# FofanovLab/mtsv_tools

Measured on AMD Instinct MI355X. Metric: reads/sec (whole node), 150bp reads vs MG-index, higher is better.
Workload: dtype u32/i16

## Files before the change

mtsv_tools_amd/csrc/dev_index.hip:

```cpp
#include <algorithm>
#include <chrono>
#include <cstdio>
#include <cstdlib>
#include <cstring>
#include <stdexcept>
#include <thread>
#include <vector>

#include "dev_index.hpp"
#include "kernels.hpp"

namespace mtsv {

void throw_hip(hipError_t e, const char* what, const char* file, int line) {
    throw std::runtime_error(std::string("device: ") + hipGetErrorString(e) + " at " + what + " (" + file + ":" +
                             std::to_string(line) + ")");
}

DeviceIndex::~DeviceIndex() {
    if (device < 0) return;
    (void)hipSetDevice(device);
    (void)hipFree(d_blocks);
    (void)hipFree(d_sa_sample);
    (void)hipFree(d_sa_full);
    (void)hipFree(d_text);
    (void)hipFree(d_bin_end);
    (void)hipFree(d_bins);
    (void)hipFree(d_bin_lut);
    (void)hipFree(d_kmer);
    (void)hipFree(d_kmer_levels);
}

namespace {

inline uint32_t sym_code(uint8_t c) {
    switch (c) {
    case 'A': return kCodeA;
    case 'C': return kCodeC;
    case 'G': return kCodeG;
    case 'T': return kCodeT;
    case 'N': return kCodeN;
    case '$': return kCodeSentinel;
    default: return 7;
    }
}


__global__ void k_expand_sa(DevIndexView ix, uint32_t n_samples, uint32_t* __restrict__ sa_full) {
    uint32_t j = blockIdx.x * blockDim.x + threadIdx.x;
    if (j >= n_samples) return;
    uint32_t row = j * ix.sa_s;
    uint32_t v = ix.sa_sample[j];
    sa_full[row] = v;
    for (uint32_t guard = 0; guard <= ix.n; guard++) {
        uint32_t blk = row >> kBlockShift, off = row & (kBlockRows - 1);
        LoadedBlock b = load_block(ix.blocks, blk);
        uint32_t c = block_code(b, off);
        if (c == kCodeSentinel) break;
        row = less_of(ix, c) + block_rank(b, c, blk, off, ix.sentinel_row);
        v -= 1;
        if (row % ix.sa_s == 0) break;
        sa_full[row] = v;
    }
}

__global__ void k_kmer_level1(DevIndexView ix, uint2* __restrict__ tab) {
    uint32_t a = threadIdx.x;
    if (a >= 4) return;
    uint32_t lo = less_of(ix, a) + dev_rank(ix, a, 0);
    uint32_t hi = less_of(ix, a) + dev_rank(ix, a, ix.n);
    tab[a] = make_uint2(lo, hi);
}

__global__ void k_kmer_level(DevIndexView ix, const uint2* __restrict__ prev, uint2* __restrict__ cur,
                             uint32_t prev_shift) {
    const uint64_t total = 4ull << prev_shift, stride = (uint64_t)gridDim.x * blockDim.x;
    for (uint64_t t = (uint64_t)blockIdx.x * blockDim.x + threadIdx.x; t < total; t += stride) {
        uint32_t a = (uint32_t)(t >> prev_shift);
        uint64_t p = t & ((1ull << prev_shift) - 1);
        uint2 iv = prev[p];
        uint32_t lo = 0, hi = 0;
        if (iv.x < iv.y) {
            uint32_t b0 = iv.x >> kBlockShift, b1 = iv.y >> kBlockShift;
            LoadedBlock B0 = load_block(ix.blocks, b0);
            lo = less_of(ix, a) + block_rank(B0, a, b0, iv.x & (kBlockRows - 1), ix.sentinel_row);
            if (b1 == b0) {
                hi = less_of(ix, a) + block_rank(B0, a, b1, iv.y & (kBlockRows - 1), ix.sentinel_row);
            } else {
                LoadedBlock B1 = load_block(ix.blocks, b1);
                hi = less_of(ix, a) + block_rank(B1, a, b1, iv.y & (kBlockRows - 1), ix.sentinel_row);
            }
        }
        cur[t] = make_uint2(lo, hi);
    }
}

__global__ void k_kmer_tag(DevIndexView ix, uint2* __restrict__ tab, uint64_t total, unsigned long long* __restrict__ n_tagged) {
    const uint64_t stride = (uint64_t)gridDim.x * blockDim.x;
    uint32_t mine = 0;
    for (uint64_t t = (uint64_t)blockIdx.x * blockDim.x + threadIdx.x; t < total; t += stride) {
        const uint2 iv = tab[t];
        if (iv.y != iv.x + 1) continue;
        const uint32_t lo = iv.x;
        const uint32_t p = ix.sa_full[lo];
        const LoadedBlock b = load_block(ix.blocks, lo >> kBlockShift);
        const uint32_t c1 = block_code(b, lo & (kBlockRows - 1));
        const uint32_t c2 = p >= 2 ? ix.text[p - 2] : 7u;
        tab[t] = kmer_tag_entry(p, c1, c2);
        mine++;
    }
    for (int d = 32; d > 0; d >>= 1) mine += __shfl_down(mine, d);
    if ((threadIdx.x & 63) == 0 && mine) atomicAdd(n_tagged, (unsigned long long)mine);
}

template <class F>
void parallel_ranges(uint64_t n, int threads, F fn) {
    std::vector<std::thread> pool;
    uint64_t chunk = (n + threads - 1) / threads;
    for (int t = 0; t < threads; t++) {
        uint64_t lo = std::min(n, (uint64_t)t * chunk), hi = std::min(n, lo + chunk);
        pool.emplace_back(fn, lo, hi, t);
    }
    for (auto& th : pool) th.join();
}

}

static void pack_on_host(const HostIndex& hx, const uint32_t n, const uint32_t n_blocks, std::vector<RankBlock>& blocks, uint64_t& sentinel_row,
                         std::vector<uint8_t>& codes) {
    int threads = (int)std::max(1u, std::min(32u, std::thread::hardware_concurrency()));
    if (n_blocks < 4096) threads = 1;

    blocks.resize(n_blocks);
    std::vector<std::array<uint64_t, 6>> range_cnt(threads);
    uint64_t blocks_per = ((uint64_t)n_blocks + threads - 1) / threads;
    parallel_ranges(n_blocks, threads, [&](uint64_t, uint64_t, int t) {
        uint64_t b0 = std::min<uint64_t>(n_blocks, (uint64_t)t * blocks_per), b1 = std::min<uint64_t>(n_blocks, b0 + blocks_per);
        std::array<uint64_t, 6> c{};
        uint64_t lo = b0 << kBlockShift, hi = std::min<uint64_t>(n, b1 << kBlockShift);
        for (uint64_t i = lo; i < hi; i++) {
            uint32_t code = sym_code(hx.bwt[i]);
            if (code < 6) c[code]++;
        }
        range_cnt[t] = c;
    });
    std::vector<std::array<uint64_t, 6>> range_base(threads);
    {
        std::array<uint64_t, 6> acc{};
        for (int t = 0; t < threads; t++) {
            range_base[t] = acc;
            for (int a = 0; a < 6; a++) acc[a] += range_cnt[t][a];
        }
    }
    std::vector<std::string> errs(threads);
    std::vector<uint64_t> sentinel_rows(threads, UINT64_MAX);
    static const uint8_t syms[6] = {'A', 'C', 'G', 'T', 'N', '$'};
    parallel_ranges(n_blocks, threads, [&](uint64_t, uint64_t, int t) {
        uint64_t b0 = std::min<uint64_t>(n_blocks, (uint64_t)t * blocks_per), b1 = std::min<uint64_t>(n_blocks, b0 + blocks_per);
        std::array<uint64_t, 6> c = range_base[t];
        for (uint64_t b = b0; b < b1; b++) {
            RankBlock rb;
            for (int a = 0; a < 4; a++) rb.cnt[a] = (uint32_t)c[a];
            uint64_t p0[2] = {0, 0}, p1[2] = {0, 0}, p2[2] = {0, 0};
            for (uint32_t o = 0; o < kBlockRows; o++) {
                uint64_t i = (b << kBlockShift) + o;
                uint32_t code = 7;
                if (i < n) {
                    code = sym_code(hx.bwt[i]);
                    if (code >= 6) {
                        errs[t] = "format: bwt holds a symbol outside ACGTN$";
                        return;
                    }
                    c[code]++;
                    if (code == kCodeSentinel) sentinel_rows[t] = i;
                    if (i % hx.k == 0) {
                        uint64_t j = i / hx.k;
                        for (int a = 0; a < 6; a++)
                            if (hx.occ[syms[a]][j] != c[a]) {
                                errs[t] = "format: Occ checkpoint " + std::to_string(j) + " disagrees with the bwt";
                                return;
                            }
                    }
                }
                p0[o >> 6] |= (uint64_t)(code & 1) << (o & 63);
                p1[o >> 6] |= (uint64_t)((code >> 1) & 1) << (o & 63);
                p2[o >> 6] |= (uint64_t)((code >> 2) & 1) << (o & 63);
            }
            rb.p0[0] = p0[0]; rb.p0[1] = p0[1];
            rb.p1[0] = p1[0]; rb.p1[1] = p1[1];
            rb.p2[0] = p2[0]; rb.p2[1] = p2[1];
            blocks[b] = rb;
        }
    });
    for (auto& e : errs)
        if (!e.empty()) throw std::runtime_error(e);
    sentinel_row = UINT64_MAX;
    for (uint64_t s : sentinel_rows)
        if (s != UINT64_MAX) sentinel_row = s;
    if (sentinel_row == UINT64_MAX) throw std::runtime_error("format: bwt holds no sentinel");

    codes.assign(((uint64_t)n + 15) / 16 * 16 + 32, (uint8_t)7);
    parallel_ranges(n, threads, [&](uint64_t lo, uint64_t hi, int) {
        for (uint64_t i = lo; i < hi; i++) codes[i] = (uint8_t)sym_code(hx.text[i]);
    });
}

namespace {
struct DevTemp {
    void* p = nullptr;
    ~DevTemp() { (void)hipFree(p); }
    void alloc(uint64_t bytes) { HIP_CHECK(hipMalloc(&p, bytes ? bytes : 16)); }
    void release() {
        HIP_CHECK(hipFree(p));
        p = nullptr;
    }
};
struct DevEvents {
    hipEvent_t e[7] = {nullptr, nullptr, nullptr, nullptr, nullptr, nullptr, nullptr};
    DevEvents() {
        for (auto& x : e) HIP_CHECK(hipEventCreate(&x));
    }
    ~DevEvents() {
        for (auto& x : e)
            if (x) (void)hipEventDestroy(x);
    }
};
}

static uint64_t pack_on_device(const HostIndex& hx, const uint32_t n, const uint32_t n_blocks, DeviceIndex& di, double& copy_ms) {
    auto now_ms = [] { return std::chrono::duration<double, std::milli>(std::chrono::steady_clock::now().time_since_epoch()).count(); };
    uint32_t tile = kPackTile;
    if (const char* e = getenv("MTSV_PACK_TILE")) {
        const int t = atoi(e);
        if (t >= 1 && t <= (int)kPackTileMax && !(t & (t - 1))) tile = (uint32_t)t;
    }
    static const uint8_t syms[6] = {'A', 'C', 'G', 'T', 'N', '$'};
    const uint64_t n_chk = ((uint64_t)n - 1) / hx.k + 1;
    for (uint8_t a : syms)
        if (hx.occ[a].size() < n_chk) throw std::runtime_error("format: occ checkpoint count != floor((n-1)/k)+1");
    const uint32_t tiles = pack_tiles(n_blocks, tile);
    const uint64_t raw_bytes = ((uint64_t)n + 15) / 16 * 16;
    DevEvents ev;
    DevTemp d_bwt, d_occ, d_tiles, d_ctr, d_raw_text;

    HIP_CHECK(hipMalloc((void**)&di.d_blocks, (uint64_t)n_blocks * sizeof(RankBlock)));
    di.bytes += (uint64_t)n_blocks * sizeof(RankBlock);
    d_bwt.alloc(raw_bytes);
    d_occ.alloc(6 * n_chk * 8);
    d_tiles.alloc((uint64_t)tiles * sizeof(uint4));
    d_ctr.alloc(kPackCounters * 4);
    uint32_t ctr[kPackCounters] = {0};
    ctr[kPackCtrForeignRow] = ctr[kPackCtrOccBadFirst] = 0xffffffffu;
    double t0 = now_ms();
    HIP_CHECK(hipMemcpy(d_bwt.p, hx.bwt.data(), n, hipMemcpyHostToDevice));
    for (int a = 0; a < 6; a++)
        HIP_CHECK(hipMemcpy((uint64_t*)d_occ.p + a * n_chk, hx.occ[syms[a]].data(), n_chk * 8, hipMemcpyHostToDevice));
    HIP_CHECK(hipMemcpy(d_ctr.p, ctr, sizeof ctr, hipMemcpyHostToDevice));
    copy_ms += now_ms() - t0;

    HIP_CHECK(hipEventRecord(ev.e[0], 0));
    launch_pack_count(0, (const uint8_t*)d_bwt.p, n, n_blocks, tile, (uint4*)d_tiles.p, (uint32_t*)d_ctr.p);
    HIP_CHECK(hipEventRecord(ev.e[1], 0));
    launch_pack_scan(0, (uint4*)d_tiles.p, tiles);
    HIP_CHECK(hipEventRecord(ev.e[2], 0));
    launch_pack_blocks(0, (const uint8_t*)d_bwt.p, n, n_blocks, tile, (const uint4*)d_tiles.p, di.d_blocks);
    HIP_CHECK(hipEventRecord(ev.e[3], 0));
    launch_pack_check_occ(0, di.d_blocks, n, hx.k, (uint32_t)n_chk, (const uint64_t*)d_occ.p, (uint32_t*)d_ctr.p);
    HIP_CHECK(hipGetLastError());
    HIP_CHECK(hipEventRecord(ev.e[4], 0));
    HIP_CHECK(hipMemcpy(ctr, d_ctr.p, sizeof ctr, hipMemcpyDeviceToHost));
    d_bwt.release();
    d_occ.release();
    d_tiles.release();
    d_ctr.release();
    const uint64_t occ_row = ctr[kPackCtrOccBad] ? (uint64_t)ctr[kPackCtrOccBadFirst] * hx.k : UINT64_MAX;
    if (ctr[kPackCtrForeign] && ctr[kPackCtrForeignRow] <= occ_row) throw std::runtime_error("format: bwt holds a symbol outside ACGTN$");
    if (ctr[kPackCtrOccBad])
        throw std::runtime_error("format: Occ checkpoint " + std::to_string(ctr[kPackCtrOccBadFirst]) + " disagrees with the bwt");
    if (!ctr[kPackCtrSentinels]) throw std::runtime_error("format: bwt holds no sentinel");

    HIP_CHECK(hipMalloc((void**)&di.d_text, di.text_bytes));
    di.bytes += di.text_bytes;
    d_raw_text.alloc(raw_bytes);
    t0 = now_ms();
    HIP_CHECK(hipMemcpy(d_raw_text.p, hx.text.data(), n, hipMemcpyHostToDevice));
    copy_ms += now_ms() - t0;
    HIP_CHECK(hipEventRecord(ev.e[5], 0));
    launch_pack_text(0, (const uint8_t*)d_raw_text.p, n, di.d_text, di.text_bytes);
    HIP_CHECK(hipGetLastError());
    HIP_CHECK(hipEventRecord(ev.e[6], 0));
    HIP_CHECK(hipEventSynchronize(ev.e[6]));
    d_raw_text.release();
    float ms[5] = {0.f, 0.f, 0.f, 0.f, 0.f};
    for (int k = 0; k < 4; k++) HIP_CHECK(hipEventElapsedTime(&ms[k], ev.e[k], ev.e[k + 1]));
    HIP_CHECK(hipEventElapsedTime(&ms[4], ev.e[5], ev.e[6]));
    di.pack_ms = ms[0] + ms[1] + ms[2] + ms[3] + ms[4];
    if (getenv("MTSV_TRACE"))
        fprintf(stderr, "[upload] pack on device, tile %u: k_pack_count %.3f k_pack_scan %.3f k_pack_blocks %.3f k_pack_check_occ %.3f k_pack_text %.3f ms\n",
                tile, ms[0], ms[1], ms[2], ms[3], ms[4]);
    return ctr[kPackCtrSentinelRow];
}

std::unique_ptr<DeviceIndex> upload_index(const HostIndex& hx, int device, uint32_t flags) {
    const uint64_t n64 = hx.n();
    if (n64 >= 0xFFFFFF00ull)
        throw std::runtime_error("limit: index of 2^32 symbols or more does not fit the u32 device layout; chunk the database (mtsv-chunk)");
    int ndev = 0;
    if (hipGetDeviceCount(&ndev) != hipSuccess || ndev <= 0)
        throw std::runtime_error("device: no HIP device visible (this library has no CPU path)");
    if (device < 0 || device >= ndev) throw std::runtime_error("device: invalid device ordinal " + std::to_string(device));
    HIP_CHECK(hipSetDevice(device));

    const uint32_t n = (uint32_t)n64;
    const uint32_t n_blocks = (n >> kBlockShift) + 1;
    const char* pack_env = getenv("MTSV_DEV_PACK");
    const bool on_device = (flags & 4u ) || (pack_env && !strcmp(pack_env, "device"));
    auto now_ms = [] { return std::chrono::duration<double, std::milli>(std::chrono::steady_clock::now().time_since_epoch()).count(); };

    std::vector<RankBlock> blocks;
    std::vector<uint8_t> codes;
    uint64_t sentinel_row = UINT64_MAX;
    const double pack_t0 = now_ms();
    if (!on_device) pack_on_host(hx, n, n_blocks, blocks, sentinel_row, codes);
    const double host_pack_ms = now_ms() - pack_t0;

    std::vector<uint32_t> samp(hx.sample.size());
    for (size_t i = 0; i < samp.size(); i++) samp[i] = (uint32_t)hx.sample[i];
    std::vector<DevBin> bins(hx.bins.size());
    std::vector<uint32_t> bin_end(hx.bins.size());
    for (size_t i = 0; i < bins.size(); i++) {
        bins[i] = DevBin{(uint32_t)hx.bins[i].start, (uint32_t)hx.bins[i].end, hx.bins[i].tax_id, hx.bins[i].gi};
        bin_end[i] = (uint32_t)hx.bins[i].end;
    }

    uint32_t lut_shift = 0;
    while (((uint64_t)n >> lut_shift) > 65536) lut_shift++;
    std::vector<uint32_t> bin_lut(((uint64_t)n >> lut_shift) + 2);
    {
        uint32_t b = 0;
        for (size_t k = 0; k < bin_lut.size(); k++) {
            uint64_t p = (uint64_t)k << lut_shift;
            while (b + 1 < bins.size() && bin_end[b] <= p) b++;
            bin_lut[k] = b;
        }
    }

    auto di = std::make_unique<DeviceIndex>();
    di->device = device;
    di->flags = flags;
    double copy_ms = 0;
    auto up = [&](auto** dptr, const void* src, uint64_t bytes) {
        HIP_CHECK(hipMalloc((void**)dptr, bytes ? bytes : 16));
        const double t0 = now_ms();
        if (bytes) HIP_CHECK(hipMemcpy(*dptr, src, bytes, hipMemcpyHostToDevice));
        copy_ms += now_ms() - t0;
        di->bytes += bytes;
    };
    di->text_bytes = ((uint64_t)n + 15) / 16 * 16 + 32;
    di->sa_sample_bytes = samp.size() * 4;
    di->bin_lut_bytes = bin_lut.size() * 4;
    di->packed_on_device = on_device;
    if (on_device) {
        sentinel_row = pack_on_device(hx, n, n_blocks, *di, copy_ms);
        up(&di->d_sa_sample, samp.data(), samp.size() * 4);
    } else {
        di->pack_ms = (float)host_pack_ms;
        up(&di->d_blocks, blocks.data(), (uint64_t)n_blocks * sizeof(RankBlock));
        up(&di->d_sa_sample, samp.data(), samp.size() * 4);
        up(&di->d_text, codes.data(), codes.size());
    }
    up(&di->d_bin_end, bin_end.data(), bin_end.size() * 4);
    up(&di->d_bins, bins.data(), bins.size() * sizeof(DevBin));
    up(&di->d_bin_lut, bin_lut.data(), bin_lut.size() * 4);

    DevIndexView& v = di->view;
    v.blocks = di->d_blocks;
    v.n = n;
    v.n_blocks = n_blocks;
    v.C[0] = (uint32_t)hx.less['A'];
    v.C[1] = (uint32_t)hx.less['C'];
    v.C[2] = (uint32_t)hx.less['G'];
    v.C[3] = (uint32_t)hx.less['T'];
    v.C[4] = (uint32_t)hx.less['N'];
    v.sentinel_row = (uint32_t)sentinel_row;
    v.sa_sample = di->d_sa_sample;
    v.sa_s = (uint32_t)hx.s;
    v.sa_pow2_shift = 0xffffffffu;
    if (hx.s > 0xFFFFFFFFull) throw std::runtime_error("limit: suffix sampling interval does not fit u32");
    for (uint32_t sh = 0; sh < 32; sh++)
        if ((1ull << sh) == hx.s) v.sa_pow2_shift = sh;
    v.sa_full = nullptr;
    v.text = di->d_text;
    v.bin_end = di->d_bin_end;
    v.bins = di->d_bins;
    v.n_bins = (uint32_t)bins.size();
    v.bin_lut = di->d_bin_lut;
    v.bin_lut_shift = lut_shift;
    v.kmer_tab = nullptr;
    v.kmer_k = 0;

    hipEvent_t e0, e1;
    HIP_CHECK(hipEventCreate(&e0));
    HIP_CHECK(hipEventCreate(&e1));
    HIP_CHECK(hipEventRecord(e0, 0));
    if (!(flags & 1u )) {
        HIP_CHECK(hipMalloc((void**)&di->d_sa_full, (uint64_t)n * 4));
        di->bytes += (uint64_t)n * 4;
        uint32_t ns = (uint32_t)samp.size();
        hipLaunchKernelGGL(k_expand_sa, dim3((ns + 255) / 256), dim3(256), 0, 0, v, ns, di->d_sa_full);
        HIP_CHECK(hipGetLastError());
        v.sa_full = di->d_sa_full;
    }
    if (!(flags & 2u )) {
        uint32_t k = 1;
        while (k < 16 && (1ull << (2 * (k + 1))) <= 2 * (uint64_t)n) k++;
        if (k == 16 && n >= (1u << 31)) k = 17;
        if (const char* e = getenv("MTSV_KMER_K")) {
            int kk = atoi(e);
            if (kk >= 1 && kk <= 17) k = (uint32_t)kk;
        }
        size_t free_b = 0, total_b = 0;
        HIP_CHECK(hipMemGetInfo(&free_b, &total_b));
        if (k == 17 && (10ull << 34) + (48ull << 30) > (uint64_t)free_b) k = 16;
        while (k > 1 && k <= 16 && (10ull << (2 * k)) * 2 > (uint64_t)free_b) k--;
        uint64_t entries = 1ull << (2 * k);
        uint2 *ta = nullptr, *tb = nullptr;
        if (k == 17) {
            if (hipMalloc((void**)&ta, entries * 8) != hipSuccess || hipMalloc((void**)&tb, entries / 4 * 8) != hipSuccess) {
                (void)hipGetLastError();
                if (ta) (void)hipFree(ta);
                ta = tb = nullptr;
                k = 16;
                entries = 1ull << 32;
            }
        }
        if (!ta) {
            HIP_CHECK(hipMalloc((void**)&ta, entries * 8));
            HIP_CHECK(hipMalloc((void**)&tb, std::max<uint64_t>(entries / 4, 4) * 8));
        }
        const char* kl = getenv("MTSV_KMER_LEVELS");
        const uint32_t n_levels = ((kl && atoi(kl) == 0) || !v.sa_full) ? 0 : std::min(k, kKmerLevelsMax);
        uint64_t level_bytes = 0;
        if (n_levels) {
            level_bytes = (uint64_t)kmer_level_start(n_levels + 1) * sizeof(uint2);
            HIP_CHECK(hipMalloc((void**)&di->d_kmer_levels, level_bytes));
            di->bytes += level_bytes;
        }
        auto keep_level = [&](uint32_t lvl, const uint2* src) {
            if (lvl <= n_levels)
                HIP_CHECK(hipMemcpyAsync(di->d_kmer_levels + kmer_level_start(lvl), src, (sizeof(uint2)) << (2 * lvl),
                                         hipMemcpyDeviceToDevice, 0));
        };
        uint2* cur = (k % 2 == 1) ? ta : tb;
        uint2* oth = (k % 2 == 1) ? tb : ta;
        hipLaunchKernelGGL(k_kmer_level1, dim3(1), dim3(64), 0, 0, v, cur);
        keep_level(1, cur);
        for (uint32_t lvl = 2; lvl <= k; lvl++) {
            const uint64_t total = 1ull << (2 * lvl);
            hipLaunchKernelGGL(k_kmer_level, dim3((uint32_t)std::min<uint64_t>((total + 255) / 256, 1u << 22)), dim3(256), 0, 0, v, cur, oth,
                               2 * (lvl - 1));
            std::swap(cur, oth);
            keep_level(lvl, cur);
        }
        HIP_CHECK(hipGetLastError());
        HIP_CHECK(hipDeviceSynchronize());
        HIP_CHECK(hipFree(tb));
        di->d_kmer = ta;
        di->bytes += entries * 8;
        v.kmer_tab = di->d_kmer;
        v.kmer_k = k;
        if (getenv("MTSV_TRACE"))
            fprintf(stderr, "[upload] kmer levels 1..%u kept: %llu bytes\n", n_levels, (unsigned long long)level_bytes);
        const char* kp = getenv("MTSV_KMER_POS");
        if (v.sa_full && !(kp && atoi(kp) == 0)) {
            unsigned long long* d_n = nullptr;
            HIP_CHECK(hipMalloc((void**)&d_n, sizeof(unsigned long long)));
            HIP_CHECK(hipMemset(d_n, 0, sizeof(unsigned long long)));
            hipEvent_t t0, t1;
            HIP_CHECK(hipEventCreate(&t0));
            HIP_CHECK(hipEventCreate(&t1));
            HIP_CHECK(hipEventRecord(t0, 0));
            hipLaunchKernelGGL(k_kmer_tag, dim3((uint32_t)std::min<uint64_t>((entries + 255) / 256, 1u << 16)), dim3(256), 0, 0, v,
                               di->d_kmer, entries, d_n);
            HIP_CHECK(hipGetLastError());
            HIP_CHECK(hipEventRecord(t1, 0));
            unsigned long long n_tagged = 0;
            HIP_CHECK(hipMemcpy(&n_tagged, d_n, sizeof(n_tagged), hipMemcpyDeviceToHost));
            float ms = 0.f;
            HIP_CHECK(hipEventElapsedTime(&ms, t0, t1));
            (void)hipEventDestroy(t0);
            (void)hipEventDestroy(t1);
            (void)hipFree(d_n);
            if (getenv("MTSV_TRACE"))
                fprintf(stderr, "[upload] kmer table k=%u: %llu tagged entries of %llu (%.1f ms)\n", k, n_tagged,
                        (unsigned long long)entries, ms);
        } else if (getenv("MTSV_TRACE")) {
            fprintf(stderr, "[upload] kmer table k=%u: 0 tagged entries of %llu (0.0 ms)\n", k, (unsigned long long)entries);
        }
    }
    HIP_CHECK(hipEventRecord(e1, 0));
    HIP_CHECK(hipEventSynchronize(e1));
    HIP_CHECK(hipEventElapsedTime(&di->accel_build_ms, e0, e1));
    (void)hipEventDestroy(e0);
    (void)hipEventDestroy(e1);
    di->copy_ms = (float)copy_ms;
    return di;
}

}
```

mtsv_tools_amd/csrc/k_verify.hip:

```cpp
#include "kernels_common.hpp"

namespace mtsv {

namespace {

typedef short pk16 __attribute__((ext_vector_type(2)));

__device__ inline pk16 pk(int lo, int hi) {
    pk16 r;
    r.x = (short)lo;
    r.y = (short)hi;
    return r;
}
__device__ inline pk16 pk_max(pk16 a, pk16 b) { return __builtin_elementwise_max(a, b); }
__device__ inline int pk_bits(pk16 a) { return __builtin_bit_cast(int, a); }
__device__ inline pk16 pk_from_bits(int u) { return __builtin_bit_cast(pk16, u); }

constexpr uint32_t kGroup = 16;
constexpr uint32_t kRing = 1024;

__device__ inline int row_shr1(int v) { return __builtin_amdgcn_update_dpp(0, v, 0x111, 0xf, 0xf, true); }

__device__ inline uint32_t group_ballot(bool p, uint32_t group) { return (uint32_t)(__ballot(p) >> (group * kGroup)) & 0xffffu; }

__device__ inline uint4 load16(const uint8_t* __restrict__ text, uint32_t n, uint32_t pos) {
    (void)n;
    const uint4* t128 = reinterpret_cast<const uint4*>(text);
    const uint32_t w = pos >> 4, dsel = (pos >> 2) & 3u, sh = pos & 3u;
    const uint4 a = t128[w], b = t128[w + 1];
    const uint32_t e0 = dsel == 0 ? a.x : dsel == 1 ? a.y : dsel == 2 ? a.z : a.w;
    const uint32_t e1 = dsel == 0 ? a.y : dsel == 1 ? a.z : dsel == 2 ? a.w : b.x;
    const uint32_t e2 = dsel == 0 ? a.z : dsel == 1 ? a.w : dsel == 2 ? b.x : b.y;
    const uint32_t e3 = dsel == 0 ? a.w : dsel == 1 ? b.x : dsel == 2 ? b.y : b.z;
    const uint32_t e4 = dsel == 0 ? b.x : dsel == 1 ? b.y : dsel == 2 ? b.z : b.w;
    uint4 r;
    r.x = __builtin_amdgcn_alignbyte(e1, e0, sh);
    r.y = __builtin_amdgcn_alignbyte(e2, e1, sh);
    r.z = __builtin_amdgcn_alignbyte(e3, e2, sh);
    r.w = __builtin_amdgcn_alignbyte(e4, e3, sh);
    return r;
}

enum : uint32_t { PH_FETCH = 0, PH_SWEEP = 1, PH_DONE = 2, PH_CHAIN = 3, PH_WAIT = 4 };

template <int R, bool WORD, int GS, bool TILED = false>
__global__ __launch_bounds__(256, (WORD || R * GS > 160) ? 1 : (GS == 8 ? 3 : 5)) void k_evaluate(DevIndexView ix, EvalArgs a) {
    static_assert(!TILED || WORD, "the tiled kernel is the long-read path: it carries the word kernel");
    __shared__ __attribute__((aligned(16))) uint8_t ring_all[256 / GS][kRing];
    const uint32_t lane = lane_id();
    const uint32_t gl = lane & (GS - 1);
    uint8_t* ring = ring_all[threadIdx.x / GS];
    uint2* strip = TILED ? a.strip + (uint64_t)(blockIdx.x * (256 / GS) + threadIdx.x / GS) * a.strip_len : nullptr;
    uint32_t band = 0, n_bands = 1;
    uint2 bnd_next = make_uint2(0, 0);
    uint32_t b0_read = 0, strand_read = 0;
    const uint32_t n_work = *a.wl_count;
    const pk16 one = pk(1, 1), miss = pk(-1, -1);
    const uint32_t maxc = a.maxc;

    uint32_t phase = PH_FETCH;
    uint32_t loc = 0, loc_end = 0;
    uint32_t g = 0, o = 0, ED = 0, thr = 0, L = 0;
    bool thr_wrapped = false, hopeless = false;
    uint32_t qc[R];
    pk16 clampRow[R];
    uint32_t t = 0, steps = 0, Wn = 0, wstart = 0, c_next = 7;
    uint32_t c_tax = 0, c_gi = 0, c_off = 0;
    pk16 h[R], up_prev = pk(0, 0), best = pk(0, -32768), last = pk(0, -32768);
    int hw[WORD ? R : 1], hwp[WORD ? R : 1];
    int upw_prev = 0, bestw = 0;
    uint32_t bmask = 0;
    unsigned long long verified = 0, wbytes = 0;
#pragma unroll
    for (int r = 0; r < R; r++) {
        qc[r] = 6;
        clampRow[r] = pk(0, 0);
        h[r] = pk(0, 0);
    }

    for (;;) {
        if (phase == PH_FETCH || phase == PH_CHAIN) {
            bool have = true;
            if (phase == PH_FETCH) {
                if (loc == loc_end) {
                    uint32_t base = 0;
                    if (gl == 0) base = atomicAdd(a.wl_cursor, 16u);
                    base = (uint32_t)__shfl((int)base, (int)(lane & ~(uint32_t)(GS - 1)));
                    loc = min(base, n_work);
                    loc_end = min(base + 16, n_work);
                }
                if (loc < loc_end) {
                    g = a.worklist[loc++];
                    const uint32_t rs = a.cand[g].w;
                    const uint32_t r_ = a.r0 + (rs >> 1), strand = rs & 1;
                    o = a.strand_off[rs];
                    const uint32_t b0 = a.read_off[r_];
                    L = a.read_off[r_ + 1] - b0;
                    ED = (uint32_t)ceil((double)L * a.edit_rate);
                    thr_wrapped = 2ull * ED > (uint64_t)L;
                    thr = L - 2 * ED;
                    const uint8_t* read = a.bases + b0;
                    if (TILED) {
                        n_bands = (L + GS * R - 1) / (GS * R);
                        b0_read = b0;
                        strand_read = strand;
                        int nn = 0;
                        for (uint32_t p = gl; p < L; p += GS) nn += strand_code(read, L, strand, p) == kCodeN;
#pragma unroll
                        for (int d = 1; d < GS; d <<= 1) nn += __shfl_xor(nn, d);
                        hopeless = thr_wrapped || (uint32_t)nn > ED;
                    } else {
                    const int pad = (int)(GS * R) - (int)L;
#pragma unroll
                    for (int r = 0; r < R; r++) {
                        int p = (int)(gl * R + r) - pad;
                        qc[r] = p >= 0 ? strand_code(read, L, strand, (uint32_t)p) : 6u;
                        clampRow[r] = p >= 0 ? pk(0, -32768) : pk(0, 0);
                    }
                    if (WORD) {
                        const int seg8 = (int)((L + 7) / 8);
                        bmask = 0;
#pragma unroll
                        for (int r = 0; r < (WORD ? R : 1); r++) {
                            int p = (int)(gl * R + r) - pad;
                            if (p >= 0 && p % seg8 == 0) bmask |= 1u << r;
                        }
                    }
                    int nn = 0;
#pragma unroll
                    for (int r = 0; r < R; r++) nn += qc[r] == kCodeN;
#pragma unroll
                    for (int d = 1; d < GS; d <<= 1) nn += __shfl_xor(nn, d);
                    hopeless = thr_wrapped || (uint32_t)nn > ED;
                    }
                } else {
                    phase = PH_DONE;
                    have = false;
                }
            }
            if (have && hopeless) {
                const uint4 c = a.cand[g];
                verified++;
                wbytes += c.y - c.x;
                if (gl == 0) a.cand_status[g] = 1;
                const uint32_t nxt = a.cand_next[g];
                if (nxt != 0xffffffffu && nxt < maxc) {
                    g = o + nxt;
                    phase = PH_CHAIN;
                } else {
                    phase = PH_FETCH;
                }
                have = false;
            }
// ... 793 lines not shown
        wave_lds_handoff();
        n = 0;
    };
    auto item_at = [&](uint32_t i) { return a.worklist[a.wl_reverse ? n_work - 1 - i : i]; };
    const uint32_t n_waves = gridDim.x * (256 / kWave), wave_g = blockIdx.x * (256 / kWave) + threadIdx.x / kWave;
    auto index_of = [&](uint32_t it) {
        return ((uint64_t)(it >> 3) * n_waves + wave_g) * 32 + (it & 7u) * 4 + (lane >> 4);
    };
    const uint32_t trips = (n_work + n_waves * 32 - 1) / (n_waves * 32) * 8;
    uint32_t gi_2 = 0, gi_1 = 0, gi_0 = 0;
    uint4 c_1 = make_uint4(0, 0, 0, 0), c_0 = c_1;
    uint32_t b0_0 = 0, L_0 = 0;
    if (index_of(2) < n_work) gi_2 = item_at((uint32_t)index_of(2));
    if (index_of(1) < n_work) {
        gi_1 = item_at((uint32_t)index_of(1));
        c_1 = a.cand[gi_1];
    }
    if (index_of(0) < n_work) {
        gi_0 = item_at((uint32_t)index_of(0));
        c_0 = a.cand[gi_0];
        const uint32_t r_ = a.r0 + (c_0.w >> 1);
        b0_0 = a.read_off[r_];
        L_0 = a.read_off[r_ + 1] - b0_0;
    }
    for (uint32_t it = 0; it < trips; it++) {
        const bool have = index_of(it) < n_work;
        uint32_t gi_3 = 0, b0_1 = 0, L_1 = 0;
        uint4 c_2 = make_uint4(0, 0, 0, 0);
        if (index_of(it + 3) < n_work) gi_3 = item_at((uint32_t)index_of(it + 3));
        if (index_of(it + 2) < n_work) c_2 = a.cand[gi_2];
        if (index_of(it + 1) < n_work) {
            const uint32_t r1 = a.r0 + (c_1.w >> 1);
            b0_1 = a.read_off[r1];
            L_1 = a.read_off[r1 + 1] - b0_1;
        }
        bool decided = false;
        const uint32_t gi = gi_0;
        if (have) {
            const uint4 c = c_0;
            const uint32_t rs = c.w;
            const uint32_t b0 = b0_0, L = L_0;
            const uint32_t ED = (uint32_t)ceil((double)L * a.edit_rate);
            const uint32_t W = c.y - c.x;
            if (gl == 0) {
                verified++;
                wbytes += W;
            }
            if (2ull * ED <= (uint64_t)L && ED + L <= W) {
                const uint32_t p0 = gl * (4 * NW);
                uint32_t rd[NW];
                {
                    const bool rev = (rs & 1u) != 0;
                    const uint32_t pq = p0 < L ? p0 : 0u;
                    const long long ba = rev ? (long long)b0 + L - 4 * NW - pq : (long long)b0 + pq;
                    const long long w = ba >> 2;
                    const uint32_t sh = (uint32_t)(ba & 3);
                    uint32_t d[NW + 1];
#pragma unroll
                    for (int k = 0; k <= NW; k++) d[k] = b32[max(w + k, 0ll)];
                    uint32_t x[NW];
#pragma unroll
                    for (int k = 0; k < NW; k++) x[k] = __builtin_amdgcn_alignbyte(d[k + 1], d[k], sh);
#pragma unroll
                    for (int k = 0; k < NW; k++) rd[k] = rev ? comp_codes4(__builtin_bswap32(x[NW - 1 - k])) : x[k];
                }
                const uint32_t pc = c.x + ED + p0;
                const uint32_t wi = pc >> 2, sc = pc & 3u;
                uint32_t wv[NW + 2];
                wv[0] = t32[wi >= 1 ? min(wi - 1, lastw) : 0u];
#pragma unroll
                for (int k = 0; k <= NW; k++) wv[k + 1] = t32[min(wi + k, lastw)];
                int ca[3][NW];
#pragma unroll
                for (int k = 0; k < NW; k++) {
                    const uint32_t lo = wv[k + 1], hi = wv[k + 2], bl = wv[k];
                    const uint32_t s0 = sc == 0 ? __builtin_amdgcn_alignbyte(lo, bl, 3u) : __builtin_amdgcn_alignbyte(hi, lo, sc - 1u);
                    const uint32_t s1 = __builtin_amdgcn_alignbyte(hi, lo, sc);
                    const uint32_t s2 = sc == 3 ? hi : __builtin_amdgcn_alignbyte(hi, lo, sc + 1u);
                    const uint32_t pk_ = p0 + 4 * k;
                    const uint32_t nv = pk_ < L ? min(L - pk_, 4u) : 0u;
                    const uint32_t valid = nv >= 4 ? 0x01010101u : ((1u << (8 * nv)) - 1u) & 0x01010101u;
                    ca[0][k] = __popc(nz_bytes(rd[k] ^ s0) & valid);
                    ca[1][k] = __popc(nz_bytes(rd[k] ^ s1) & valid);
                    ca[2][k] = __popc(nz_bytes(rd[k] ^ s2) & valid);
                }
                int mm[3];
#pragma unroll
                for (int d = 0; d < 3; d++) {
                    mm[d] = 0;
#pragma unroll
                    for (int k = 0; k < NW; k++) mm[d] += ca[d][k];
                }
                decided = (uint32_t)row_sum16(mm[1]) <= ED;
                if (!decided && ED >= 1 && ED + L + 1 <= W) {
                    int below[3], above[3];
#pragma unroll
                    for (int d = 0; d < 3; d++) {
                        below[d] = row_prefix_incl16(mm[d]) - mm[d];
                        above[d] = row_suffix_incl16(mm[d]) - mm[d];
                    }
                    auto split = [&](int da, int db) {
                        int pa = 0, sb = mm[db], best = mm[db];
#pragma unroll
                        for (int k = 0; k < NW; k++) {
                            pa += ca[da][k];
                            sb -= ca[db][k];
                            best = min(best, pa + sb);
                        }
                        return below[da] + best + above[db];
                    };
                    int best = min(min(split(1, 0), split(1, 2)), min(split(0, 1), split(2, 1)));
                    best = -row_max16(-best);
                    decided = best <= (int)ED - 1;
                }
            }
        }
        const unsigned long long pm = __ballot(have && gl == 0 && decided), sm = __ballot(have && gl == 0 && !decided);
        const unsigned long long lower = (1ull << lane) - 1ull;
        if (have && gl == 0 && decided) pbuf[np + (uint32_t)__popcll(pm & lower)] = gi;
        if (have && gl == 0 && !decided) sbuf[nsw + (uint32_t)__popcll(sm & lower)] = gi;
        np += (uint32_t)__popcll(pm);
        nsw += (uint32_t)__popcll(sm);
        if (np + 4 > kDiagBuf) flush(pbuf, np, sw_pass_count(a), a.pass_list, 0u);
        if (nsw + 4 > kDiagBuf) flush(sbuf, nsw, reinterpret_cast<uint32_t*>(a.counters + sweep_slot), sweep_list, kSweepFlag);
        gi_0 = gi_1;
        gi_1 = gi_2;
        gi_2 = gi_3;
        c_0 = c_1;
        c_1 = c_2;
        b0_0 = b0_1;
        L_0 = L_1;
    }
    if (np) flush(pbuf, np, sw_pass_count(a), a.pass_list, 0u);
    if (nsw) flush(sbuf, nsw, reinterpret_cast<uint32_t*>(a.counters + sweep_slot), sweep_list, kSweepFlag);
    for (int d = 32; d > 0; d >>= 1) {
        verified += __shfl_down(verified, d);
        wbytes += __shfl_down(wbytes, d);
    }
    if (lane == 0 && verified) {
        atomicAdd((unsigned long long*)a.counters + kCtrVerified, verified);
        atomicAdd((unsigned long long*)a.counters + kCtrWindowBytes, wbytes);
    }
}

__device__ inline uint32_t clamp_codes4(uint32_t x) {
    const uint32_t t = x & 0x04040404u;
    return t | (x & 0x03030303u & ~((t >> 1) | (t >> 2)));
}
__device__ inline uint32_t clamp_codes_sw(uint32_t x) {
    const uint32_t t = x & 0x04040404u, lo = x & 0x03030303u;
    const uint32_t nz = (lo | (lo >> 1)) & 0x01010101u, m = t >> 2;
    return t | (lo & ~(m * 3u)) | ((nz ^ 0x01010101u) & m);
}
__device__ inline uint4 fetch_cols(const DevIndexView& ix, uint32_t start, uint32_t end, uint32_t strand, uint32_t j0, bool sw_matches) {
    uint4 r;
    if (!strand) {
        r = load16(ix.text, ix.n, start + j0);
    } else if (end >= j0 + 16) {
        const uint4 v = load16(ix.text, ix.n, end - j0 - 16);
        r.x = __builtin_amdgcn_perm(0, v.w, 0x00010203u);
        r.y = __builtin_amdgcn_perm(0, v.z, 0x00010203u);
        r.z = __builtin_amdgcn_perm(0, v.y, 0x00010203u);
        r.w = __builtin_amdgcn_perm(0, v.x, 0x00010203u);
    } else {
        uint32_t w[4] = {0, 0, 0, 0};
        for (uint32_t i = 0; i < 16; i++) {
            const uint32_t code = end >= j0 + 1 + i ? ix.text[end - j0 - 1 - i] : 7u;
            w[i >> 2] |= code << (8 * (i & 3));
        }
        r = make_uint4(w[0], w[1], w[2], w[3]);
    }
    r.x = sw_matches ? clamp_codes_sw(r.x) : clamp_codes4(r.x);
    r.y = sw_matches ? clamp_codes_sw(r.y) : clamp_codes4(r.y);
    r.z = sw_matches ? clamp_codes_sw(r.z) : clamp_codes4(r.z);
    r.w = sw_matches ? clamp_codes_sw(r.w) : clamp_codes4(r.w);
    return r;
}

enum : int { MY_CHAIN = 0, MY_LIST = 1, MY_BOUND = 2, MY_FUSED = 3 };
template <int W, int MODE>
__global__ __launch_bounds__(256) void k_edit_myers(DevIndexView ix, EvalArgs a) {
    constexpr bool FUSED = MODE == MY_FUSED, LIST = MODE == MY_LIST || FUSED, BOUND = MODE == MY_BOUND;
    constexpr int NROW = (BOUND || LIST) ? 6 : 5;
    __shared__ uint32_t eq_tab[NROW][W][256];
    const uint32_t tid = threadIdx.x;
    const uint32_t n_work = *a.wl_count;
    const uint32_t maxc = a.maxc;
    const uint32_t lane = lane_id();
    uint32_t verified = 0, wbytes = 0;
    uint32_t cols = 0, refuted = 0;
    uint32_t bnext = 0, bend = 0;
    bool active = false, exhausted = false;
    bool counted = false;
    uint32_t g = 0, o = 0, L = 0, ED = 0, strand = 0;
    bool thr_wrapped = false, hopeless = false;
    uint32_t pv0[W];
    uint32_t ph = 0, extra_passed = 0;
    bool read_n = false;
    for (;;) {
        unsigned long long need = __ballot(!active);
        if (need) {
            if (bnext == bend && !exhausted) {
                const uint32_t n_waves = gridDim.x * (256 / kWave);
                const uint32_t claim = min(256u, max(64u, (n_work / n_waves + 63u) & ~63u));
                uint32_t base = 0;
                if (lane == 0) base = atomicAdd(a.wl_cursor, claim);
                base = __builtin_amdgcn_readfirstlane(base);
                bnext = min(base, n_work);
                bend = min(base + claim, n_work);
                exhausted = bnext == bend;
            }
            const uint32_t take = bnext + __popcll(need & ((1ull << lane) - 1));
            if (!active && take < bend) {
                g = a.worklist[FUSED && a.wl_reverse ? n_work - 1 - take : take];
                if (BOUND) {
                    counted = (g & kSweepFlag) != 0;
                    g &= ~kSweepFlag;
                }
                const uint32_t rs = a.cand[g].w;
                const uint32_t r_ = a.r0 + (rs >> 1);
                strand = rs & 1;
                o = a.strand_off[rs];
                const uint32_t b0 = a.read_off[r_];
                L = a.read_off[r_ + 1] - b0;
                ED = (uint32_t)ceil((double)L * a.edit_rate);
                thr_wrapped = 2ull * ED > (uint64_t)L;
                const int pad = 32 * W - (int)L;
                const uint32_t nw = (L + 31) >> 5, pw = (uint32_t)(pad + 31) >> 5, sh = (uint32_t)(-pad) & 31u;
                const uint32_t* img = a.planes + ((uint64_t)(rs >> 1) * a.plane_words) * 3;
                uint32_t P0[W + 1], P1[W + 1], PN[W + 1];
#pragma unroll
                for (int j = 0; j <= W; j++) {
                    const uint32_t idx = (uint32_t)j - pw;
                    P0[j] = P1[j] = PN[j] = 0;
                    if (idx < nw) {
                        P0[j] = img[3 * idx];
                        P1[j] = img[3 * idx + 1];
                        PN[j] = img[3 * idx + 2];
                    }
                }
                uint32_t read_ns = 0;
#pragma unroll
                for (int k = 0; k < W; k++) {
                    const uint32_t p0 = __builtin_amdgcn_alignbit(P0[k + 1], P0[k], sh), p1 = __builtin_amdgcn_alignbit(P1[k + 1], P1[k], sh),
                                   pn = __builtin_amdgcn_alignbit(PN[k + 1], PN[k], sh);
                    const int below = pad - 32 * k;
                    const uint32_t wild = below >= 32 ? 0xffffffffu : below <= 0 ? 0u : (1u << below) - 1u;
                    const uint32_t mA = ~(p0 | p1 | pn), mC = (p0 & ~p1 & ~pn) | wild, mG = (p1 & ~p0 & ~pn) | wild,
                                   mT = (p0 & p1 & ~pn) | wild;
                    read_ns += __popc(pn);
                    eq_tab[0][k][tid] = strand ? mT : mA;
                    eq_tab[1][k][tid] = strand ? mG : mC;
                    eq_tab[2][k][tid] = strand ? mC : mG;
                    eq_tab[3][k][tid] = strand ? mA : mT;
                    eq_tab[4][k][tid] = wild;
                    if (NROW == 6) eq_tab[5][k][tid] = pn | wild;
                    pv0[k] = ~wild;
                }
                hopeless = thr_wrapped || (!BOUND && read_ns > ED);
                read_n = read_ns != 0;
                ph = FUSED ? 1 : 0;
                active = true;
            }
            bnext = min(bnext + (uint32_t)__popcll(need), bend);
        }
        if (!__any(active)) {
            if (exhausted) break;
            continue;
        }
        uint32_t verdict = 0, vg = 0;
        if ((FUSED ? thr_wrapped : !LIST && hopeless) && active) {
            const uint4 c = a.cand[g];
            if (!BOUND || !counted) {
                verified++;
                wbytes += c.y - c.x;
            }
            counted = false;
            a.cand_status[g] = 1;
            const uint32_t nxt = a.cand_next[g];
            if (nxt == 0xffffffffu || nxt >= maxc) active = false;
            else g = o + nxt;
        } else if (active) {
            const uint4 c = a.cand[g];
            uint32_t Pv[W], Mv[W];
#pragma unroll
            for (int k = 0; k < W; k++) {
                Pv[k] = pv0[k];
                Mv[k] = 0;
            }
            const uint32_t Wn = c.y - c.x;
            int score = (int)L, best = (int)L;
            const bool swm = BOUND || (LIST && ph == 1);
            uint4 nxt4 = Wn ? fetch_cols(ix, c.x, c.y, strand, 0, swm) : make_uint4(0, 0, 0, 0);
            const uint32_t* lane_tab = &eq_tab[0][0][tid];
            uint32_t j0 = 0;
            uint32_t win_n = 0;
            for (; j0 < Wn; j0 += 16) {
                if (swm) {
                    if (BOUND && best <= (int)ED) break;
                    if (best > 2 * (int)ED && score - (int)(Wn - j0) > 2 * (int)ED) break;
                }
                const uint4 cur = nxt4;
                if (LIST) win_n |= cur.x | cur.y | cur.z | cur.w;
                if (j0 + 16 < Wn) nxt4 = fetch_cols(ix, c.x, c.y, strand, j0 + 16, swm);
                const uint32_t lim = min(16u, Wn - j0);
#pragma unroll
                for (int jj = 0; jj < 16; jj++) {
                    if ((uint32_t)jj < lim) {
                        const uint32_t word = jj < 4 ? cur.x : jj < 8 ? cur.y : jj < 12 ? cur.z : cur.w;
                        const uint32_t tc = (word >> ((jj & 3) * 8)) & 0xffu;
                        const uint32_t* row = lane_tab + tc * (W * 256);
                        uint32_t ph_below = 0, mh_below = 0;
#pragma unroll
                        for (int k = 0; k < W; k++) {
                            const uint32_t Eq = row[k * 256];
                            const uint32_t pv = Pv[k], mv = Mv[k];
                            const uint32_t Xv = Eq | mv;
                            const uint32_t Eqh = k ? (Eq | (mh_below >> 31)) : Eq;
                            const uint32_t Xh = __builtin_amdgcn_bitop3_b32((Eqh & pv) + pv, pv, Eqh, 0xBE);
                            const uint32_t Ph = mv | ~(Xh | pv);
                            const uint32_t Mh = pv & Xh;
                            const uint32_t Phs = k ? __builtin_amdgcn_alignbit(Ph, ph_below, 31) : (Ph << 1);
                            const uint32_t Mhs = k ? __builtin_amdgcn_alignbit(Mh, mh_below, 31) : (Mh << 1);
                            Pv[k] = Mhs | ~(Xv | Phs);
                            Mv[k] = Phs & Xv;
                            ph_below = Ph;
                            mh_below = Mh;
                        }
                        const uint32_t hp = ph_below >> 31, hm = mh_below >> 31;
                        score += (int)hp - (int)hm;
                        best = min(best, score);
                    }
                }
            }
            cols += min(j0, Wn);
            if (LIST ? ph == 1 : (!BOUND || !counted)) {
                verified++;
                wbytes += Wn;
            }
            counted = false;
            const uint32_t ed = (uint32_t)best;
            if (BOUND) {
                if (!thr_wrapped && ed <= ED) {
                    verdict = 1;
                    vg = g;
                    active = false;
                } else if (!thr_wrapped && ed <= 2 * ED) {
                    verdict = 2;
                    vg = g;
                    active = false;
                } else {
                    refuted++;
                    a.cand_status[g] = 1;
                    const uint32_t nxt = a.cand_next[g];
                    if (nxt == 0xffffffffu || nxt >= maxc) active = false;
                    else g = o + nxt;
                }
            } else if (LIST && ph == 1) {
                if (ed > 2 * ED) {
                    if (FUSED) refuted++;
                    a.cand_status[g] = 1;
                    const uint32_t nxt = a.cand_next[g];
                    if (nxt == 0xffffffffu || nxt >= maxc) active = false;
                    else g = o + nxt;
                } else if (ed > ED) {
                    if (FUSED) {
                        verdict = 2;
                    } else {
                        a.next_list[atomicAdd(a.next_count, 1u)] = g | kSweepFlag;
                    }
                    active = false;
                } else {
                    extra_passed++;
                    if (!read_n || !(win_n & 0x04040404u)) {
                        const DevBin bin = ix.bins[c.z];
                        a.out[g] = make_uint4(bin.tax_id, bin.gi, c.x >= bin.start ? c.x - bin.start : 0, ed);
                        a.cand_status[g] = 2;
                        active = false;
                    } else {
                        ph = 2;
                    }
                }
            } else {
            const bool pass = !thr_wrapped && ed <= ED;
            if (pass) {
                const DevBin bin = ix.bins[c.z];
                a.out[g] = make_uint4(bin.tax_id, bin.gi, c.x >= bin.start ? c.x - bin.start : 0, ed);
                a.cand_status[g] = 2;
                active = false;
            } else {
                a.cand_status[g] = 1;
                const uint32_t nxt = a.cand_next[g];
                if (nxt == 0xffffffffu || nxt >= maxc) active = false;
                else {
                    g = o + nxt;
                    if (LIST) ph = 1;
                }
            }
            }
        }
        if (BOUND || FUSED) {
            const unsigned long long pm = BOUND ? __ballot(verdict == 1) : 0ull, um = __ballot(verdict == 2);
            const unsigned long long lower = (1ull << lane) - 1ull;
            if (pm) {
                uint32_t base = 0;
                if (lane == 0) base = atomicAdd(sw_pass_count(a), (uint32_t)__popcll(pm));
                base = __builtin_amdgcn_readfirstlane(base);
                if (verdict == 1) a.pass_list[base + (uint32_t)__popcll(pm & lower)] = vg;
            }
            if (um) {
                uint32_t base = 0;
                if (lane == 0) base = atomicAdd(reinterpret_cast<uint32_t*>(a.counters + a.und_slot), (uint32_t)__popcll(um));
                base = __builtin_amdgcn_readfirstlane(base);
                if (verdict == 2) a.und_list[base + (uint32_t)__popcll(um & lower)] = (FUSED ? g : vg) | kSweepFlag;
            }
        }
    }
    unsigned long long v64 = verified, w64 = wbytes;
    for (int d = 32; d > 0; d >>= 1) {
        v64 += __shfl_down(v64, d);
        w64 += __shfl_down(w64, d);
    }
    if (lane == 0 && v64) {
        atomicAdd(a.n_verified, v64);
        atomicAdd(a.window_bytes, w64);
    }
    if (a.myers_ctr) {
        unsigned long long c64 = cols, r64 = refuted;
        for (int d = 32; d > 0; d >>= 1) {
            c64 += __shfl_down(c64, d);
            r64 += __shfl_down(r64, d);
        }
        unsigned long long e64 = extra_passed;
        for (int d = 32; d > 0; d >>= 1) e64 += __shfl_down(e64, d);
        if (lane == 0) {
            atomicAdd(a.myers_ctr, c64);
            if ((BOUND || FUSED) && r64) atomicAdd(a.myers_ctr + 1, r64);
            if (LIST && e64) atomicAdd(a.myers_ctr + 2, e64);
        }
    }
}

__global__ __launch_bounds__(256) void k_resolve(uint32_t n_strands, int64_t max_candidates, int64_t max_assignments,
                                                 const uint32_t* __restrict__ strand_off,
                                                 const uint32_t* __restrict__ strand_ncand,
                                                 const uint32_t* __restrict__ cand_status, uint4* __restrict__ out,
                                                 uint32_t* __restrict__ strand_nout) {
    const uint32_t rs = blockIdx.x * blockDim.x + threadIdx.x;
    const bool valid = rs < n_strands;
    uint32_t nc = valid ? strand_ncand[rs] : 0;
    uint32_t nout = 0;
    const uint32_t o = nc ? strand_off[rs] : 0;
    if (max_candidates >= 0 && (uint64_t)nc > (uint64_t)max_candidates) nc = (uint32_t)max_candidates;
    constexpr uint32_t kCoop = 32;
    const bool big = nc > kCoop;
    if (nc && !big) {
        for (uint32_t i = 0; i < nc; i++) {
            if (cand_status[o + i] == 2) {
                if (nout != i) out[o + nout] = out[o + i];
                nout++;
                if (max_assignments >= 0 && (uint64_t)nout >= (uint64_t)max_assignments) break;
            }
        }
    }
    const uint32_t lane = lane_id();
    const uint64_t cap = max_assignments < 0 ? ~0ull : (uint64_t)(max_assignments > 1 ? max_assignments : 1);
    for (unsigned long long m = __ballot(big); m; m &= m - 1) {
        const int l = __builtin_ctzll(m);
        const uint32_t o_l = __builtin_amdgcn_readlane(o, l), nc_l = __builtin_amdgcn_readlane(nc, l);
        uint32_t nout_l = 0;
        for (uint32_t base = 0; base < nc_l; base += kWave) {
            const uint32_t i = base + lane;
            const bool pass = i < nc_l && cand_status[o_l + i] == 2;
            uint4 v = make_uint4(0, 0, 0, 0);
            if (pass) v = out[o_l + i];
            const unsigned long long pm = __ballot(pass);
            const uint32_t pos = nout_l + (uint32_t)__popcll(pm & ((1ull << lane) - 1));
            if (pass && (uint64_t)pos < cap) out[o_l + pos] = v;
            nout_l += (uint32_t)__popcll(pm);
            if ((uint64_t)nout_l >= cap) {
                nout_l = (uint32_t)cap;
                break;
            }
        }
        if ((int)lane == l) nout = nout_l;
    }
// ... 146 lines not shown
```

Baseline: 444.9 million.

## Stream Myers verify text through aligned 128-bit chunk register ring

Replaces the per-16-column unaligned fetch (with a byte-by-byte fallback for reverse-strand edges) with a window stream. It issues aligned 16-byte loads of the padded text in groups of four chunks, keeps them in a register ring, and builds each column block with perm/alignbyte. The intent is to turn scattered unaligned global loads and the slow scalar tail path into fewer aligned vector loads issued ahead of use. The cost is extra registers for the five-chunk ring, which may reduce occupancy, and loads that can run past early-exit points. The text padding is recomputed through a shared helper so the aligned loads stay in bounds.

```diff
diff --git a/mtsv_tools_amd/csrc/dev_index.hip b/mtsv_tools_amd/csrc/dev_index.hip
--- a/mtsv_tools_amd/csrc/dev_index.hip
+++ b/mtsv_tools_amd/csrc/dev_index.hip
@@ -9,6 +9,7 @@
 
 #include "dev_index.hpp"
 #include "kernels.hpp"
+#include "window_stream.hpp"
 
 namespace mtsv {
 
@@ -199,7 +200,7 @@
         if (s != UINT64_MAX) sentinel_row = s;
     if (sentinel_row == UINT64_MAX) throw std::runtime_error("format: bwt holds no sentinel");
 
-    codes.assign(((uint64_t)n + 15) / 16 * 16 + 32, (uint8_t)7);
+    codes.assign((uint64_t)text_chunks((uint32_t)n) * 16, (uint8_t)7);
     parallel_ranges(n, threads, [&](uint64_t lo, uint64_t hi, int) {
         for (uint64_t i = lo; i < hi; i++) codes[i] = (uint8_t)sym_code(hx.text[i]);
     });
@@ -356,7 +357,7 @@
         copy_ms += now_ms() - t0;
         di->bytes += bytes;
     };
-    di->text_bytes = ((uint64_t)n + 15) / 16 * 16 + 32;
+    di->text_bytes = (uint64_t)text_chunks((uint32_t)n) * 16;
     di->sa_sample_bytes = samp.size() * 4;
     di->bin_lut_bytes = bin_lut.size() * 4;
     di->packed_on_device = on_device;
diff --git a/mtsv_tools_amd/csrc/k_verify.hip b/mtsv_tools_amd/csrc/k_verify.hip
--- a/mtsv_tools_amd/csrc/k_verify.hip
+++ b/mtsv_tools_amd/csrc/k_verify.hip
@@ -1,4 +1,5 @@
 #include "kernels_common.hpp"
+#include "window_stream.hpp"
 
 namespace mtsv {
 
@@ -1098,31 +1099,6 @@
     const uint32_t nz = (lo | (lo >> 1)) & 0x01010101u, m = t >> 2;
     return t | (lo & ~(m * 3u)) | ((nz ^ 0x01010101u) & m);
 }
-__device__ inline uint4 fetch_cols(const DevIndexView& ix, uint32_t start, uint32_t end, uint32_t strand, uint32_t j0, bool sw_matches) {
-    uint4 r;
-    if (!strand) {
-        r = load16(ix.text, ix.n, start + j0);
-    } else if (end >= j0 + 16) {
-        const uint4 v = load16(ix.text, ix.n, end - j0 - 16);
-        r.x = __builtin_amdgcn_perm(0, v.w, 0x00010203u);
-        r.y = __builtin_amdgcn_perm(0, v.z, 0x00010203u);
-        r.z = __builtin_amdgcn_perm(0, v.y, 0x00010203u);
-        r.w = __builtin_amdgcn_perm(0, v.x, 0x00010203u);
-    } else {
-        uint32_t w[4] = {0, 0, 0, 0};
-        for (uint32_t i = 0; i < 16; i++) {
-            const uint32_t code = end >= j0 + 1 + i ? ix.text[end - j0 - 1 - i] : 7u;
-            w[i >> 2] |= code << (8 * (i & 3));
-        }
-        r = make_uint4(w[0], w[1], w[2], w[3]);
-    }
-    r.x = sw_matches ? clamp_codes_sw(r.x) : clamp_codes4(r.x);
-    r.y = sw_matches ? clamp_codes_sw(r.y) : clamp_codes4(r.y);
-    r.z = sw_matches ? clamp_codes_sw(r.z) : clamp_codes4(r.z);
-    r.w = sw_matches ? clamp_codes_sw(r.w) : clamp_codes4(r.w);
-    return r;
-}
-
 enum : int { MY_CHAIN = 0, MY_LIST = 1, MY_BOUND = 2, MY_FUSED = 3 };
 template <int W, int MODE>
 __global__ __launch_bounds__(256) void k_edit_myers(DevIndexView ix, EvalArgs a) {
@@ -1237,18 +1213,37 @@
             const uint32_t Wn = c.y - c.x;
             int score = (int)L, best = (int)L;
             const bool swm = BOUND || (LIST && ph == 1);
-            uint4 nxt4 = Wn ? fetch_cols(ix, c.x, c.y, strand, 0, swm) : make_uint4(0, 0, 0, 0);
+            const WindowStream ws = window_stream(c.x, c.y, strand, ix.n);
+            const uint32_t osel = stream_selector(strand);
+            const uint4* t128 = reinterpret_cast<const uint4*>(ix.text);
+            auto load_chunk = [&](uint32_t i) {
+                uint4 v = make_uint4(0x07070707u, 0x07070707u, 0x07070707u, 0x07070707u);
+                if (i < ws.lim) v = t128[stream_text_chunk(ws, i)];
+                return stream_orient(wchunk{v.x, v.y, v.z, v.w}, osel);
+            };
+            auto clamp_cols = [&](const wchunk& r) {
+                return make_uint4(swm ? clamp_codes_sw(r.x) : clamp_codes4(r.x), swm ? clamp_codes_sw(r.y) : clamp_codes4(r.y),
+                                  swm ? clamp_codes_sw(r.z) : clamp_codes4(r.z), swm ? clamp_codes_sw(r.w) : clamp_codes4(r.w));
+            };
+            StreamRegs sr;
+            stream_prime(sr, load_chunk);
+            uint4 nxt4 = clamp_cols(stream_cols(sr.ch[0], sr.ch[1], ws.off));
             const uint32_t* lane_tab = &eq_tab[0][0][tid];
             uint32_t j0 = 0;
             uint32_t win_n = 0;
-            for (; j0 < Wn; j0 += 16) {
+            bool more = Wn != 0;
+            while (more) {
+#pragma unroll
+            for (uint32_t bi = 0; bi < kStreamGroup; bi++) {
                 if (swm) {
-                    if (BOUND && best <= (int)ED) break;
-                    if (best > 2 * (int)ED && score - (int)(Wn - j0) > 2 * (int)ED) break;
+                    if ((BOUND && best <= (int)ED) || (best > 2 * (int)ED && score - (int)(Wn - j0) > 2 * (int)ED)) {
+                        more = false;
+                        break;
+                    }
                 }
                 const uint4 cur = nxt4;
                 if (LIST) win_n |= cur.x | cur.y | cur.z | cur.w;
-                if (j0 + 16 < Wn) nxt4 = fetch_cols(ix, c.x, c.y, strand, j0 + 16, swm);
+                nxt4 = clamp_cols(stream_next_cols(sr, ws.off, bi, load_chunk));
                 const uint32_t lim = min(16u, Wn - j0);
 #pragma unroll
                 for (int jj = 0; jj < 16; jj++) {
@@ -1278,6 +1273,12 @@
                         best = min(best, score);
                     }
                 }
+                j0 += 16;
+                if (j0 >= Wn) {
+                    more = false;
+                    break;
+                }
+            }
             }
             cols += min(j0, Wn);
             if (LIST ? ph == 1 : (!BOUND || !counted)) {
diff --git a/mtsv_tools_amd/csrc/window_stream.hpp b/mtsv_tools_amd/csrc/window_stream.hpp
--- /dev/null
+++ b/mtsv_tools_amd/csrc/window_stream.hpp
@@ -0,0 +1,128 @@
+#pragma once
+#include <cstdint>
+
+#if defined(__HIPCC__) || defined(__CUDACC__)
+#define MTSV_WS_HD __host__ __device__
+#else
+#define MTSV_WS_HD
+#endif
+
+namespace mtsv {
+
+constexpr uint32_t kTextPadChunks = 2;
+constexpr uint32_t kStreamGroup = 4;
+
+struct wchunk {
+    uint32_t x, y, z, w;
+};
+
+struct WindowStream {
+    uint32_t base;
+    uint32_t off;
+    uint32_t lim;
+    uint32_t strand;
+};
+
+MTSV_WS_HD inline uint32_t text_chunks(uint32_t n) { return (n >> 4) + ((n & 15u) ? 1u : 0u) + kTextPadChunks; }
+
+MTSV_WS_HD inline WindowStream window_stream(uint32_t start, uint32_t end, uint32_t strand, uint32_t n) {
+    WindowStream ws;
+    ws.strand = strand;
+    const uint32_t wn = end - start, blocks = (wn + 15u) >> 4, total = text_chunks(n);
+    if (!strand) {
+        ws.base = start >> 4;
+        ws.off = start & 15u;
+    } else {
+        ws.base = (end - 1u) >> 4;
+        ws.off = 15u - ((end - 1u) & 15u);
+    }
+    const uint32_t need = (ws.off + 16u * blocks + 15u) >> 4;
+    const uint32_t have = ws.base >= total ? 0u : strand ? ws.base + 1u : total - ws.base;
+    ws.lim = wn ? (need < have ? need : have) : 0u;
+    return ws;
+}
+
+MTSV_WS_HD inline uint32_t stream_text_chunk(const WindowStream& ws, uint32_t i) { return ws.strand ? ws.base - i : ws.base + i; }
+
+MTSV_WS_HD inline int stream_issue_block(uint32_t i) {
+    return i <= kStreamGroup ? -1 : (int)((i - kStreamGroup - 1u) / kStreamGroup * kStreamGroup + kStreamGroup - 2u);
+}
+
+MTSV_WS_HD inline uint32_t stream_selector(uint32_t strand) { return strand ? 0x04050607u : 0x03020100u; }
+
+MTSV_WS_HD inline uint32_t perm_bytes(uint32_t hi, uint32_t lo, uint32_t sel) {
+#if defined(__HIP_DEVICE_COMPILE__)
+    return __builtin_amdgcn_perm(hi, lo, sel);
+#else
+    const uint64_t both = ((uint64_t)hi << 32) | lo;
+    uint32_t r = 0;
+    for (int k = 0; k < 4; k++) r |= (uint32_t)((both >> (8 * ((sel >> (8 * k)) & 7u))) & 0xffu) << (8 * k);
+    return r;
+#endif
+}
+
+MTSV_WS_HD inline uint32_t align_bytes(uint32_t hi, uint32_t lo, uint32_t sh) {
+#if defined(__HIP_DEVICE_COMPILE__)
+    return __builtin_amdgcn_alignbyte(hi, lo, sh);
+#else
+    return (uint32_t)((((uint64_t)hi << 32) | lo) >> (8 * (sh & 3u)));
+#endif
+}
+
+MTSV_WS_HD inline wchunk stream_orient(const wchunk& v, uint32_t sel) {
+    wchunk r;
+    r.x = perm_bytes(v.w, v.x, sel);
+    r.y = perm_bytes(v.z, v.y, sel);
+    r.z = perm_bytes(v.y, v.z, sel);
+    r.w = perm_bytes(v.x, v.w, sel);
+    return r;
+}
+
+MTSV_WS_HD inline wchunk stream_cols(const wchunk& a, const wchunk& b, uint32_t off) {
+    const uint32_t dsel = off >> 2, sh = off & 3u;
+    const uint32_t e0 = dsel == 0 ? a.x : dsel == 1 ? a.y : dsel == 2 ? a.z : a.w;
+    const uint32_t e1 = dsel == 0 ? a.y : dsel == 1 ? a.z : dsel == 2 ? a.w : b.x;
+    const uint32_t e2 = dsel == 0 ? a.z : dsel == 1 ? a.w : dsel == 2 ? b.x : b.y;
+    const uint32_t e3 = dsel == 0 ? a.w : dsel == 1 ? b.x : dsel == 2 ? b.y : b.z;
+    const uint32_t e4 = dsel == 0 ? b.x : dsel == 1 ? b.y : dsel == 2 ? b.z : b.w;
+    wchunk r;
+    r.x = align_bytes(e1, e0, sh);
+    r.y = align_bytes(e2, e1, sh);
+    r.z = align_bytes(e3, e2, sh);
+    r.w = align_bytes(e4, e3, sh);
+    return r;
+}
+
+struct StreamRegs {
+    wchunk ch[kStreamGroup + 1];
+    uint32_t first;
+};
+
+template <class Load>
+MTSV_WS_HD inline void stream_prime(StreamRegs& s, Load&& load) {
+    s.first = 0;
+#ifdef __HIP_DEVICE_COMPILE__
+#pragma unroll
+#endif
+    for (uint32_t q = 0; q <= kStreamGroup; q++) s.ch[q] = load(q);
+}
+
+template <class Load>
+MTSV_WS_HD inline void stream_refill(StreamRegs& s, Load&& load) {
+    s.first += kStreamGroup;
+    s.ch[0] = s.ch[kStreamGroup];
+#ifdef __HIP_DEVICE_COMPILE__
+#pragma unroll
+#endif
+    for (uint32_t q = 1; q <= kStreamGroup; q++) s.ch[q] = load(s.first + q);
+}
+
+template <class Load>
+MTSV_WS_HD inline wchunk stream_next_cols(StreamRegs& s, uint32_t off, uint32_t i, Load&& load) {
+    const uint32_t p = (i + 1u) % kStreamGroup;
+    const wchunk r = stream_cols(s.ch[p], s.ch[p + 1u], off);
+    if (i == kStreamGroup - 2u) stream_refill(s, load);
+    return r;
+}
+
+}
```

After: 452.4 million, median of 4. 1.02x the previous value.
